# THUDM/GRAND-plus

Measured on AMD Instinct MI355X. Metric: propagation-matrix rows/sec (whole node), higher is better.
Workload: dtype f64

## Files before the change

### grand_plus_amd/csrc/gfpush.hip

```cpp
#include "gfpush_kernels.hpp"
#include "gfpush_sketch.hpp"
#include "gfpush_plan.hpp"
#include "grandplus.h"

#include <dlfcn.h>
#include <sys/prctl.h>
#include <rccl/rccl.h>

#include <algorithm>
#include <atomic>
#include <cmath>
#include <cstdarg>
#include <cstdio>
#include <cstdlib>
#include <cstring>
#include <new>
#include <string>
#include <chrono>
#include <thread>
#include <type_traits>
#include <vector>

using namespace gp;
using namespace gp::planning;
// ... 508 lines not shown
        if (rc == GP_ERR_NOMEM && sk.use && !shape.insists_on_sketch()) {
            sk.use = false; g_last_error.clear();
            continue;
        }
        return rc;
    }
}

KParams call_params(const gp_graph* g, const CallArgs& a, const GeneralPlan& gk, u64* counters)
{
    KParams kp;
    std::memset(&kp, 0, sizeof kp);
    kp.indptr = g->d_indptr; kp.indices = g->d_indices; kp.n_nodes = (int)g->n_nodes; kp.nnz = (int)g->nnz;
    kp.deg_shift = g->deg_shift; kp.node_mask = g->node_mask; kp.deg_sat = g->deg_sat;
    kp.seeds = a.d_seeds; kp.n_seeds = a.n_seeds;
    kp.coef = g->d_coef; kp.n_coef = a.n_coef; kp.rmax = a.rmax; kp.K = a.K;
    kp.out_row = a.d_row; kp.out_col = a.d_col; kp.out_val = a.d_val; kp.out_filled = a.d_filled;
    kp.counters = counters;
    kp.lds_slots = gk.lds_slots;
    kp.force_global = g->opt.force_global;
    kp.prune = prune_allowed(g->opt, a.coef, a.n_coef) ? 1 : 0;
    kp.diag_flags = g->opt.diag_flags;
    kp.rows_distinct = g->rows_distinct && g->opt.seedrow ? 1u : 0u;
    kp.solo = (g->opt.solo_levels ? 1u : 0u) | (g->opt.sk_seed_merge ? 2u : 0u);
    kp.direct = direct_tables(g->opt, g->n_nodes, gk) ? 1 : 0;
    return kp;
}

struct GeneralPass { const u32* rows; int n_rows; int queue; u32* overflow; int n_overflow; int overflow_queue; const u32* order; };

int launch_general(const gp_graph* g, KParams& kp, const GeneralPlan& gk, bool gk_acsr, const GeneralPass& pass, hipStream_t s)
{
    const Workspace& w = g->ws;
    const bool two_tier = w.big.n_wg > 0;
    use_csr(kp, g, gk_acsr, true);
    use_slabs(kp, w.est);
    kp.row_map = pass.rows ? pass.rows : pass.order; kp.n_rows_dev = pass.rows ? kp.counters + pass.n_rows : nullptr; kp.queue_counter = pass.queue;
    kp.retry_list = two_tier ? pass.overflow : nullptr; kp.retry_counter = pass.n_overflow;
    const Kernel k = pass.rows ? retry_kernel(gk.block_threads) : general_kernel(gk.block_threads);
    int rc = launch_kernel(k, gk.block_threads, kp, gk.n_wg, gk.lds_bytes + g->opt.lds_pad, s);
    if (rc || !two_tier) return rc;
    use_slabs(kp, w.big);
    kp.row_map = pass.overflow; kp.n_rows_dev = kp.counters + pass.n_overflow; kp.queue_counter = pass.overflow_queue;
    kp.retry_list = nullptr;
    return launch_kernel(retry_kernel(gk.block_threads), gk.block_threads, kp, w.big.n_wg, gk.lds_bytes + g->opt.lds_pad, s);
}

// ... 383 lines not shown
    if (k == "block_threads") {
        if (value != 256 && value != 512 && value != 768 && value != 1024) return fail(GP_ERR_INVALID_ARG, "block_threads must be 256, 512, 768 or 1024");
        g->opt.block_threads = (int)value;
    } else if (k == "lds_bytes") {
        if (value < 40 * 1024 || value > 160 * 1024) return fail(GP_ERR_INVALID_ARG, "lds_bytes must be in [40960, 163840]");
        g->opt.lds_bytes = (int)(value & ~15ll);
    } else if (k == "lds_pad") {
        if (value < 0 || value > 120 * 1024) return fail(GP_ERR_INVALID_ARG, "lds_pad must be in [0, 122880]");
        g->opt.lds_pad = (int)(value & ~15ll);
    } else if (k == "kernel") {
        if (value < 0 || value > 2) return fail(GP_ERR_INVALID_ARG, "kernel must be 0 (automatic), 1 (general) or 2 (sketch)");
        g->opt.kernel = (int)value;
    } else if (k == "sk_block_threads") {
        if (value != 0 && value != 512 && value != 768 && value != 1024) return fail(GP_ERR_INVALID_ARG, "sk_block_threads must be 0, 512, 768 or 1024");
        g->opt.sk_block = (int)value;
    } else if (k == "sk_lg_mu" || k == "sk_lg_mr") {
        if (value != 0 && (value < 8 || value > 14)) return fail(GP_ERR_INVALID_ARG, "%s must be 0 or in [8, 14]", key);
        (k == "sk_lg_mu" ? g->opt.sk_lg_mu : g->opt.sk_lg_mr) = (int)value;
    } else if (k == "sk_direct_max") {
        if (value < 0 || value > (1 << 20)) return fail(GP_ERR_INVALID_ARG, "sk_direct_max must be in [0, 2^20]");
        g->opt.sk_direct_max = (int)value;
    } else if (k == "sk_seed_merge") {
        g->opt.sk_seed_merge = value ? 1 : 0;
    } else if (k == "row_order") {
        g->opt.row_order = value ? 1 : 0;
    } else if (k == "gk_acsr") {
        g->opt.gk_acsr = value ? 1 : 0;
    } else if (k == "sk_target") {
        if (value < 0 || value > 4096) return fail(GP_ERR_INVALID_ARG, "sk_target must be in [0, 4096]");
        g->opt.sk_target = (int)value;
    } else if (k == "measure_choice") {
        g->opt.measure_choice = value ? 1 : 0;
        if (!value) g->choices.clear();
    } else if (k == "verify_merge") {
        g->opt.verify_merge = value ? 1 : 0;
    } else if (k == "pretouch") {
        g->opt.pretouch = value ? 1 : 0;
    } else if (k == "max_workgroups") {
        if (value < 0 || value > 65535) return fail(GP_ERR_INVALID_ARG, "max_workgroups must be in [0, 65535]");
        g->opt.max_workgroups = (int)value;
    } else if (k == "workspace_mb") {
        if (value < 1) return fail(GP_ERR_INVALID_ARG, "workspace_mb must be >= 1");
        g->opt.workspace_mb = value;
    } else if (k == "est_level_edges") {
        if (value < 0) return fail(GP_ERR_INVALID_ARG, "est_level_edges must be >= 0");
        g->opt.est_level_edges = value;
// ... 230 lines not shown
}

namespace {

int replicate_part(gp_graph* g, int d) {
    gp_graph* src = g->part[0];
    HIP_TRY(hipSetDevice(src->device));
    int rc = ensure_packed(src, src->stream);
    if (rc) return rc;
    HIP_TRY(hipStreamSynchronize(src->stream));
    const int dev = g->devices[d];
    HIP_TRY(hipSetDevice(dev));
    hipDeviceProp_t prop;
    HIP_TRY(hipGetDeviceProperties(&prop, dev));
    gp_graph* q = new (std::nothrow) gp_graph();
    if (!q) return fail(GP_ERR_NOMEM, "host allocation failed");
    struct Guard { gp_graph* q; ~Guard() { if (q) gp_graph_destroy(q); } } guard{q};
    q->device = dev; q->n_nodes = src->n_nodes; q->nnz = src->nnz; q->num_cus = prop.multiProcessorCount;
    q->deg_shift = src->deg_shift; q->node_mask = src->node_mask; q->deg_sat = src->deg_sat;
    q->packed = true; q->opt.max_degree_bits = src->opt.max_degree_bits; q->rows_distinct = src->rows_distinct;
    q->opt.block_threads = src->opt.block_threads; q->opt.lds_bytes = src->opt.lds_bytes; q->opt.max_workgroups = src->opt.max_workgroups;
    q->opt.workspace_mb = src->opt.workspace_mb; q->opt.force_global = src->opt.force_global; q->opt.exact_stats = src->opt.exact_stats;
    q->opt.direct_tables = src->opt.direct_tables; q->opt.est_level_edges = src->opt.est_level_edges; q->opt.seedrow = src->opt.seedrow; q->opt.solo_levels = src->opt.solo_levels;
    q->opt.kernel = src->opt.kernel; q->opt.row_order = src->opt.row_order; q->opt.gk_acsr = src->opt.gk_acsr; q->opt.sk_seed_merge = src->opt.sk_seed_merge; q->opt.sk_block = src->opt.sk_block; q->opt.sk_lg_mu = src->opt.sk_lg_mu; q->opt.sk_lg_mr = src->opt.sk_lg_mr; q->opt.sk_target = src->opt.sk_target; q->opt.lds_pad = src->opt.lds_pad; q->opt.sk_direct_max = src->opt.sk_direct_max;
    const size_t b_ptr = sizeof(int) * (size_t)(q->n_nodes + 1), b_idx = sizeof(int) * (size_t)(q->nnz + 1);
    HIP_TRY(hipMalloc(&q->d_indptr, b_ptr));
    HIP_TRY(hipMalloc(&q->d_indices, b_idx));
    if (dev == src->device) {
        HIP_TRY(hipMemcpy(q->d_indptr, src->d_indptr, b_ptr, hipMemcpyDeviceToDevice));
        HIP_TRY(hipMemcpy(q->d_indices, src->d_indices, b_idx, hipMemcpyDeviceToDevice));
    } else {
        HIP_TRY(hipMemcpyPeer(q->d_indptr, dev, src->d_indptr, src->device, b_ptr));
        HIP_TRY(hipMemcpyPeer(q->d_indices, dev, src->d_indices, src->device, b_idx));
    }
    HIP_TRY(hipMalloc(&q->d_counters, sizeof(u64) * kNumCounters));
    HIP_TRY(hipHostMalloc(&q->h_counters, sizeof(u64) * kNumCounters));
    HIP_TRY(hipEventCreate(&q->ev0));
    HIP_TRY(hipEventCreate(&q->ev1));
    HIP_TRY(hipStreamCreateWithFlags(&q->stream, hipStreamNonBlocking));
    guard.q = nullptr;
    g->part[d] = q;
    return GP_OK;
}

int gfpush_multi(gp_graph* g, const int32_t* seeds, int64_t n_seeds, const double* coef, int n_coef, double rmax, int K,
                 int32_t* row_idx, int32_t* col_idx, double* value)
{
// ... 114 lines not shown
```

### grand_plus_amd/csrc/gfpush_kernels.hpp

```cpp
#pragma once

#include <hip/hip_runtime.h>
#include <stdint.h>

#include "gfpush_hash.hpp"

namespace gp {

typedef unsigned long long u64;
typedef unsigned int u32;

#define GP_LDS  __attribute__((address_space(3)))
#define GP_KARG __attribute__((address_space(4)))
template <class T> __device__ __forceinline__ T* lds_at(u32 byte_off) { return (T*)(GP_LDS T*)(uintptr_t)byte_off; }
__device__ __forceinline__ u32 uni(u32 x) { return (u32)__builtin_amdgcn_readfirstlane((int)x); }
__device__ __forceinline__ int uni(int x) { return __builtin_amdgcn_readfirstlane(x); }
__device__ __forceinline__ u64 uni(u64 x) { return ((u64)uni((u32)(x >> 32)) << 32) | uni((u32)x); }
__device__ __forceinline__ long long uni(long long x) { return (long long)uni((u64)x); }
__device__ __forceinline__ double uni(double x) {
    const u64 b = (u64)__double_as_longlong(x);
    return __longlong_as_double((long long)(((u64)uni((u32)(b >> 32)) << 32) | uni((u32)b)));
}

constexpr int    kEmpty      = -1;
// ... 110 lines not shown
    x += (u32)__builtin_amdgcn_update_dpp(0, (int)x, 0x143, 0xC, 0xF, false);
    return x;
}
__device__ __forceinline__ u32 wave_id() { return (u32)__builtin_amdgcn_readfirstlane((int)(threadIdx.x >> 6)); }
__device__ __forceinline__ u32 wave_sum32(u32 x) {
    return (u32)__builtin_amdgcn_readlane((int)wave_incl_scan_dpp(x), 63);
}

enum Counter { kQueue = 0, kQueueRetry, kRetryRows,
               kQueueRetry2, kRetryRows2,
               kSkSlabFails,
               kMaxLevelEdges, kMaxLogRecords,
               kRetriedTotal,
               kPushes, kEdges, kFilled, kSupport, kFrontier, kLdsLevels,
               kGlobalLevels, kFailedRows, kDegLookups,
               kSkCandEdges, kSkSweep2,
               kTicksScan, kTicksExpand, kTicksTopk, kTicksTotal, kTicksScanHbm, kTicksExpandHbm,
               kDiag0, kDiagLast = kDiag0 + 15,
               kDiagX0, kDiagXLast = kDiagX0 + 255,
               kNumCounters };

enum OvfCount { kOvfLevel = 8,
                kOvfSolo = 9,
                kOvfTopk = 10 };
#if !defined(GP_DIAG) && !defined(GP_SK_TIMING)
#define GP_OVF_COUNT(p, which) __hip_atomic_fetch_add(&(p).counters[kDiag0 + (which)], 1ull, __ATOMIC_RELAXED, __HIP_MEMORY_SCOPE_AGENT)
#else
#define GP_OVF_COUNT(p, which) do { } while (0)
#endif

#ifdef GP_DIAG_HEAVY
constexpr int kSyncBase = __COUNTER__;
#define GP_SYNC() do { constexpr int site_ = (__COUNTER__ - kSyncBase - 1) & 63; const u64 tb_ = clock64(); __syncthreads(); if ((threadIdx.x & 63) == 0) { const u64 w_ = clock64() - tb_; ctl->barw[threadIdx.x >> 6] += w_; ++ctl->barn[threadIdx.x >> 6]; \
    __hip_atomic_fetch_add(&ctl->site_w[site_], w_, __ATOMIC_RELAXED, __HIP_MEMORY_SCOPE_WORKGROUP); __hip_atomic_fetch_add(&ctl->site_n[site_], 1u, __ATOMIC_RELAXED, __HIP_MEMORY_SCOPE_WORKGROUP); } } while (0)
#else
#define GP_SYNC() __syncthreads()
#endif
#ifdef GP_DIAG
#define GP_STAMP(var) do { if (threadIdx.x == 0) var = wall_clock64(); } while (0)
#define GP_ACCUM(acc, t0, t1) do { if (threadIdx.x == 0) acc += (t1) - (t0); } while (0)
#define GP_SUB_BEGIN() do { if (threadIdx.x == 0) gp_sub_t = wall_clock64(); } while (0)
#define GP_SUB(i) do { if (threadIdx.x == 0) { const u64 n_ = wall_clock64(); gp_sub_acc[i] += n_ - gp_sub_t; gp_sub_t = n_; } } while (0)
#define GP_SUB_COUNT(i, n) do { if (threadIdx.x == 0) gp_sub_acc[i] += (n); } while (0)
#else
#define GP_STAMP(var) do { } while (0)
#define GP_ACCUM(acc, t0, t1) do { } while (0)
#define GP_SUB_BEGIN() do { } while (0)
// ... 315 lines not shown
              [se0] "=&v"(se0), [se1] "=&v"(se1), [se2] "=&v"(se2), [se3] "=&v"(se3),
              [sv] "=&s"(sv), [m0] "=&s"(m0), [m1] "=&s"(m1), [m2] "=&s"(m2), [m3] "=&s"(m3), [st] "=&s"(st)
            : [c0] "v"(col[0]), [c1] "v"(col[1]), [c2] "v"(col[2]), [c3] "v"(col[3]), [s0] "v"(sh[0]), [s1] "v"(sh[1]), [s2] "v"(sh[2]), [s3] "v"(sh[3]),
              [emp] "v"(kEmpty), [parts] "s"(parts), [part] "s"(part),
              [capm] "s"(cap - kProbeSpan), [kb] "s"(lds_addr(keys)), [vb] "s"(lds_addr(vals)), [fa] "s"(lds_addr(flag)), [lim] "n"(kMaxProbe)
            : "vcc", "scc", "memory");
    } else {
        u64 ent;
        asm volatile(
            "s_mov_b64 %[sv], exec\n\t"
            GP_IW4_HASHES
            GP_IW4_EACH(GP_IW4_ISSUE_C)
            GP_IW4_RESOLVE_C(0, 3) GP_IW4_RESOLVE_C(1, 2) GP_IW4_RESOLVE_C(2, 1) GP_IW4_RESOLVE_C(3, 0)
            : [sl0] "=&v"(sl0), [sl1] "=&v"(sl1), [sl2] "=&v"(sl2), [sl3] "=&v"(sl3),
              [se0] "=&v"(se0), [se1] "=&v"(se1), [se2] "=&v"(se2), [se3] "=&v"(se3),
              [sv] "=&s"(sv), [ent] "=&s"(ent), [st] "=&s"(st)
            : [c0] "v"(col[0]), [c1] "v"(col[1]), [c2] "v"(col[2]), [c3] "v"(col[3]), [s0] "v"(sh[0]), [s1] "v"(sh[1]), [s2] "v"(sh[2]), [s3] "v"(sh[3]),
              [emp] "v"(kEmpty),
              [capm] "s"(cap - kProbeSpan), [kb] "s"(lds_addr(keys)), [vb] "s"(lds_addr(vals)), [fa] "s"(lds_addr(flag)), [lim] "n"(kMaxProbe)
            : "vcc", "scc", "memory");
    }
}


#define GP_IW2_EACH(X) X(0) X(1)
__device__ __forceinline__ void insert_windows2_asm(int* keys, double* vals, u32 cap, u32* flag, int c0, int c1, double s0, double s1)
{
    u32 sl0, sl1, se0, se1, st; u64 sv, ent;
    asm volatile(
        "s_mov_b64 %[sv], exec\n\t"
        GP_IW2_EACH(GP_IW4_H1) GP_IW2_EACH(GP_IW4_H2) GP_IW2_EACH(GP_IW4_H3) GP_IW2_EACH(GP_IW4_H4)
        GP_IW2_EACH(GP_IW4_ISSUE_C)
        GP_IW4_RESOLVE_C(0, 1) GP_IW4_RESOLVE_C(1, 0)
        : [sl0] "=&v"(sl0), [sl1] "=&v"(sl1), [se0] "=&v"(se0), [se1] "=&v"(se1), [sv] "=&s"(sv), [ent] "=&s"(ent), [st] "=&s"(st)
        : [c0] "v"(c0), [c1] "v"(c1), [s0] "v"(s0), [s1] "v"(s1), [emp] "v"(kEmpty),
          [capm] "s"(cap - kProbeSpan), [kb] "s"(lds_addr(keys)), [vb] "s"(lds_addr(vals)), [fa] "s"(lds_addr(flag)), [lim] "n"(kMaxProbe)
        : "vcc", "scc", "memory");
}

struct SerialSection {
    __device__ __forceinline__ SerialSection() { __builtin_amdgcn_s_setprio(3); }
    __device__ __forceinline__ ~SerialSection() { __builtin_amdgcn_s_setprio(0); }
};

__device__ __forceinline__ void insert_window_solo(int* keys, double* vals, u32 cap, u32* flag, int col, double sh, u32& slot, int& seen)
{
// ... 1772 lines not shown
```

### grand_plus_amd/csrc/gfpush_plan.hpp

```cpp
#pragma once

#include <algorithm>
#include <atomic>
#include <cmath>
#include <cstddef>
#include <cstdint>
#include <cstdio>
#include <cstring>
#include <string>

namespace gp {
namespace planning {

typedef unsigned long long cap_t;

enum Status { kOk = 0, kInvalidArg, kNoMem, kNeedOccupancy };

struct KernelConsts {
    int ctl_bytes = 0, three_lds = 0, min_cap = 0, topk_bins = 0, bucket_cap = 0, unit_shift = 0;
    int sk_max_pushers = 0, sk_max_coef = 0, sk_tie = 0;
};

struct Options {
    int block_threads = 0; int lds_bytes = 0; int max_workgroups = 0;
    int verify_merge = 0;
    int lds_pad = 0; int pretouch = 0;
    int64_t workspace_mb = 65536; int force_global = 0; int exact_stats = 0; int diag_flags = 0; int direct_tables = 1; int seedrow = 1; int solo_levels = 1;
    int kernel = 0;
    int sk_block = 0, sk_lg_mu = 0, sk_lg_mr = 0, sk_target = 0, sk_direct_max = 0;
    int row_order = 1;
    int sk_seed_merge = 1; int gk_acsr = 1;
    int64_t est_level_edges = 0;
    int measure_choice = 1;
    int max_degree_bits = 31;
};

struct Estimate {
    int kind = 0; int last_kind = 1;
    bool sk_auto_off = false; double sk_off_rmax = 0.0; int sk_off_n_coef = 0;
    bool last_sk_soft = false;
    double edges = 0.0, log = 0.0;
    double rmax = -1.0; int n_coef = 0;
    bool recipe_changed = false;
    double cur_edges = 0.0, cur_log = 0.0;
    int64_t last_call_rows = 0; bool grown_for_call = true;
};


struct SlabCaps {
    int n_wg = 0;
    cap_t push_cap = 0, resg_cap = 0, log_cap = 0, cand_cap = 0, bucket_cap = 0, bt_cap = 0;
    cap_t arch_cap = 0;
    size_t log_bytes() const { return arch_cap ? 6 * (size_t)log_cap + 8 * (size_t)arch_cap : 12 * (size_t)log_cap; }
    size_t per_wg() const { return 16 * (size_t)(2 * push_cap + resg_cap + cand_cap + bucket_cap) + log_bytes() + 8 * (size_t)bt_cap + 64; }
// ... 431 lines not shown
```

### grand_plus_amd/csrc/gfpush_sketch.hpp

```cpp
#pragma once

#include "gfpush_kernels.hpp"

#ifndef GP_DIAG

namespace gp {

#ifndef GP_SK_SWEEP_DEPTH
#define GP_SK_SWEEP_DEPTH 2
#endif
constexpr int kSkMaxCoef = 40;
constexpr u32 kSkTie     = 256;

struct CtlS {
    long long row;
    LevelCtr lc[2];
    u32 ovf;
    u32 fail;
    u32 n_sel, n_tie;
    u32 tk_bin, tk_above, tk_count, tk_total;
    u32 tk_t, tk_wide, tk_dig;
    u64 kth_bits;
    u32 bcnt[64];
    u64 st[8], st_row[8];
    double coef[kSkMaxCoef + 1];
    u32 cand_q[kSkMaxCoef];
    int seed_key; u32 tot_pu, tot_log;
    double lv_dang; u32 lv_has_dang;
    u32 max_e, max_log;
    u32 k_log_cap, k_pu_cap, k_direct_max, k_solo_ok, k_cx, k_pad; double k_rscale;
#ifdef GP_SK_TIMING
    u64 tacc[16]; u64 tlast;
    u64 tacc2[14]; u64 tlast2;
    u64 t_enter, t_row, row_sum, row_max;
    u64 row_hist[32];
#endif
};
#ifdef GP_SK_TIMING
#define SKT_BEGIN(ctl) do { if (threadIdx.x == 0) (ctl)->tlast = wall_clock64(); } while (0)
#define SKT(ctl, i) do { if (threadIdx.x == 0) { const u64 n_ = wall_clock64(); (ctl)->tacc[i] += n_ - (ctl)->tlast; (ctl)->tlast = n_; } } while (0)
#define SKT_COUNT(ctl, i, n) do { if (threadIdx.x == 0) (ctl)->tacc[i] += (n); } while (0)
#define SKT2_BEGIN(ctl) do { if (threadIdx.x == 0) (ctl)->tlast2 = wall_clock64(); } while (0)
#define SKT2(ctl, i) do { if (threadIdx.x == 0) { const u64 n_ = wall_clock64(); (ctl)->tacc2[i] += n_ - (ctl)->tlast2; (ctl)->tlast2 = n_; } } while (0)
#else
#define SKT_BEGIN(ctl) do { } while (0)
#define SKT(ctl, i) do { } while (0)
#define SKT_COUNT(ctl, i, n) do { } while (0)
#define SKT2_BEGIN(ctl) do { } while (0)
#define SKT2(ctl, i) do { } while (0)
#endif
static_assert(sizeof(CtlS) <= (size_t)kCtlStruct, "the control block must fit its LDS reservation");
enum StatS { zPush = 0, zEdges, zDeg, zFilled, zLevels, zFailed, zCand, zSweep2, zNumStats };
__device__ __forceinline__ void zstat(CtlS* ctl, int which, u64 n) {
// ... 107 lines not shown
        const u32 i = min(g0 + 4u * lane, last_chunk);
        if (NT) { kn = __builtin_nontemporal_load((const i4*)&lk[i]); pn = __builtin_nontemporal_load((const u2*)&lp[i]); }
        else    { kn = *(const i4*)&lk[i]; pn = *(const u2*)&lp[i]; }
    };
    load(g);
    for (;;) {
        int k[4]; u32 pu[4];
        const u32 i0 = g + 4u * lane;
        const bool whole = g >= first && g + 256u <= end;
        if (whole) {
#pragma unroll
            for (int q = 0; q < 4; ++q) { k[q] = kn[q]; pu[q] = (pn[q >> 1] >> (16 * (q & 1))) & 0xFFFFu; }
        } else {
#pragma unroll
            for (int q = 0; q < 4; ++q) {
                const bool in = i0 + (u32)q >= first && i0 + (u32)q < end;
                k[q] = in ? kn[q] : -1;
                pu[q] = in ? (pn[q >> 1] >> (16 * (q & 1))) & 0xFFFFu : 0u;
            }
        }
        g += kStride;
        const bool more = g < end;
        if (more) load(g);
        if (whole) f(k, pu, SkAllValid<true>()); else f(k, pu, SkAllValid<false>());
        if (!more) break;
    }
}

template <int BLOCK, class F>
__device__ __forceinline__ void log_groups2_nt(const int* lk, const unsigned short* lp, u32 end, F f)
{
    typedef int i4 __attribute__((ext_vector_type(4)));
    typedef u32 u2 __attribute__((ext_vector_type(2)));
    constexpr u32 kStride = (BLOCK / 64) * 256u;
    const u32 lane = threadIdx.x & 63u;
    u32 g = wave_id() * 256u;
    if (g >= end) return;
    const u32 last_chunk = (end - 1u) & ~3u;
    i4 ka, kb; u2 pa, pb;
    auto load = [&](u32 g0, i4& kn, u2& pn) {
        const u32 i = min(g0 + 4u * lane, last_chunk);
        kn = __builtin_nontemporal_load((const i4*)&lk[i]); pn = __builtin_nontemporal_load((const u2*)&lp[i]);
    };
    auto consume = [&](u32 g0, const i4& kn, const u2& pn, int (&k)[4], u32 (&pu)[4]) -> bool {
        const u32 i0 = g0 + 4u * lane;
        const bool whole = g0 + 256u <= end;
        if (whole) {
#pragma unroll
            for (int q = 0; q < 4; ++q) { k[q] = kn[q]; pu[q] = (pn[q >> 1] >> (16 * (q & 1))) & 0xFFFFu; }
        } else {
#pragma unroll
            for (int q = 0; q < 4; ++q) {
                const bool in = i0 + (u32)q < end;
                k[q] = in ? kn[q] : -1;
                pu[q] = in ? (pn[q >> 1] >> (16 * (q & 1))) & 0xFFFFu : 0u;
            }
        }
        return whole;
    };
    load(g, ka, pa);
    kb = ka; pb = pa;
    if (g + kStride < end) load(g + kStride, kb, pb);
    for (;;) {
        int k[4]; u32 pu[4];
        consume(g, ka, pa, k, pu);
        if (g + 2u * kStride < end) load(g + 2u * kStride, ka, pa);
        f(k, pu, SkAllValid<false>());
        g += kStride;
        if (g >= end) break;
        consume(g, kb, pb, k, pu);
        if (g + 2u * kStride < end) load(g + 2u * kStride, kb, pb);
        f(k, pu, SkAllValid<false>());
        g += kStride;
        if (g >= end) break;
    }
}

template <int BLOCK, bool NT, int FX, class F>
__device__ __forceinline__ void sk_edge_stream(KP p, CtlS* ctl, const PushEntry* push, const u32* bt, u32 n_ent, u32 E, double* S,
                                               unsigned short* lp, u32 pu_base, double cs, F f)
{
    constexpr u32 kWaves = BLOCK / 64;
    static_assert(kFlatW == 4, "sk_edge_stream reads the four window flags of a lane as one 32-bit word");
    const u32 lane = threadIdx.x & 63u;
    const u32 wave = wave_id();
    unsigned char* wscr = (unsigned char*)ctl + kCtlStruct + 64 * kFlatW * wave;
    const int* indices = p.indices;
    const u32 sentinel = (u32)p.nnz;
    const u32 units = (E + (1u << kUnitShift) - 1u) >> kUnitShift;
    const u32 slot = kWaves - 1u - wave;
    const u32 u_lo = (slot * units) / kWaves, u_hi = ((slot + 1u) * units) / kWaves;
    if (u_lo >= u_hi || n_ent == 0) return;
    const bool small = n_ent <= 64u;
    u32 btv = 0, bt_first = 0;
    auto load_bt = [&](u32 step0) {
// ... 152 lines not shown
        const double dang = w.ctl->lv_dang; const int seed_key = w.ctl->seed_key;
        if (MODE != 3) {
            lk[E] = seed_key; lp[E] = (unsigned short)(pu_base + n_ent);
            const u32 h = sk_cell((u32)seed_key);
            if (cs != 0.0) lds_add_u32(&w.R[h >> w.shR], fx_up(dang * cs));
            if (MODE == 0) { lds_add_u32(&w.U[h >> w.shU], fx_up(dang * 2147483648.0)); S[n_ent] = dang; }
        }
        if ((MODE == 1 || (MODE == 3 && (parts == 1u || slot_of(hash_b((u32)seed_key), parts) == part))) &&
            !sk_res_add_lds(w.xkeys, w.xvals, capx, seed_key, dang)) w.ctl->ovf = 1;
    }
}

template <int BLOCK>
__device__ GP_PHASE_NOINLINE void phase_sk_filter(u32 lds0, u32 seg_base, u32 n, u32 capx, u32 pu_base, u32 parts, u32 part)
{
    KP p = kparams();
    lds0 = uni(lds0); seg_base = uni(seg_base); n = uni(n); capx = uni(capx); pu_base = uni(pu_base); parts = uni(parts); part = uni(part);
    const SkView w = sk_view<BLOCK>(p, lds0);
    const float thr = p.sk_thr_f;
    const u32 dshift = (u32)p.deg_shift;
    const double* S = w.xvals + capx;
    u32 n_cand = 0;
    SKT2(w.ctl, 0);
    log_groups<BLOCK>(w.log_key, w.log_pu, seg_base, seg_base + n, [&](const int (&k)[4], const u32 (&pu)[4], auto all_valid) {
        constexpr bool kAll = decltype(all_valid)::value;
        u32 cell[4]; double s[4];
#pragma unroll
        for (int q = 0; q < 4; ++q) {
            cell[q] = w.U[sk_cell(kAll ? (u32)k[q] : (u32)max(k[q], 0)) >> w.shU];
            s[q] = S[kAll || k[q] >= 0 ? pu[q] - pu_base : 0u];
        }
        int kc[4];
#pragma unroll
        for (int q = 0; q < 4; ++q) {
            const u32 dq = (u32)k[q] >> dshift;
            const bool cand = (kAll || k[q] >= 0) && (float)cell[q] >= (float)dq * thr;
            n_cand += (u32)__popcll(__ballot(cand));
            kc[q] = cand ? k[q] : -1;
        }
        insert_windows4_asm<true>(w.xkeys, w.xvals, capx, &w.ctl->ovf, kc, s, parts, part);
    });
    if ((threadIdx.x & 63u) == 0 && n_cand && part == 0u) zstat(w.ctl, zCand, n_cand);
    SKT2(w.ctl, 1);
}

template <int BLOCK>
__device__ GP_PHASE_NOINLINE void phase_sk_scan(u32 lds0, u32 cap, u32 nx_sel, u32 nxt_sel, u32 clear_n, u32 pu_next, double cnext)
// ... 344 lines not shown
                if (__ballot(kk[j] != kEmpty && v[j] > 0.0) == 0) continue;
                bool is_sel = false, is_t = false;
                Cand cd; cd.bits = (u64)__double_as_longlong(v[j]); cd.key = kk[j]; cd.pad = 0;
                if (kk[j] != kEmpty && v[j] > 0.0) {
                    const u32 id = (u32)cd.key & p.node_mask;
                    const u64 vbits = cd.bits >> vshift;
                    const bool v_eq = vbits == vpre;
                    const bool in_bin = v_eq && (ishift >= 32u || (id >> ishift) == ipre);
                    const bool over = vbits > vpre || (v_eq && ishift < 32u && (id >> ishift) < ipre);
                    is_sel = over || (in_bin && take_all); is_t = in_bin && !take_all;
                }
                const u32 si = wave_alloc1(&ctl->n_sel, is_sel, lane);
                if (is_sel) t.sel[si] = cd;
                const u32 ti = wave_alloc1(&ctl->n_tie, is_t, lane);
                if (is_t) t.tie[ti] = cd;
            }
        }
    }
    GP_SYNC();
    sk_rank_selected<BLOCK>(p, ctl, t, need, take_all, my_rank);
    return need;
}

template <int BLOCK, bool TG>
__device__ GP_PHASE_NOINLINE void phase_sk_topk(u32 lds0, u32 row_lo, u32 row_hi, int seed, u32 n_pu, u32 n_log)
{
    KP p = kparams();
    lds0 = uni(lds0); row_lo = uni(row_lo); row_hi = uni(row_hi); seed = uni(seed); n_pu = uni(n_pu); n_log = uni(n_log);
    const SkView w = sk_view<BLOCK>(p, lds0);
    CtlS* ctl = w.ctl;
    const SkTop t = sk_top(p, w, TG ? 0u : n_pu);
    const long long row = (long long)(((u64)row_hi << 32) | row_lo);
    const int tid = threadIdx.x, lane = tid & 63;
    const u32 wave = wave_id();
    const u32 K = (u32)p.K;

    if (!TG) for (u32 i = tid; i < n_pu; i += BLOCK) t.T[i] = w.arch[i];
    for (u32 i = tid; i < 512u; i += BLOCK) t.fine[i] = 0;
    for (u32 i = tid; i < t.CA; i += BLOCK) { t.akeys[i] = kEmpty; t.avals[i] = 0.0; }
    if (tid < 64) ctl->bcnt[tid] = 0;
    if (tid == 0) { ctl->ovf = 0; ctl->tk_t = 1u; ctl->n_sel = 0; ctl->n_tie = 0; ctl->tk_wide = 0; ctl->kth_bits = ~0ull; }
    bool table_ready = true;
    GP_SYNC();
    for (u32 i = tid; i < t.MR; i += BLOCK) {
        const u32 cv = t.R[i];
        if (cv) {
            const u32 fb = __float_as_uint((float)cv);
            lds_add_u32(&t.fine[min(511u, (fb >> 19) - (127u << 4))], 1u);
        }
    }
    GP_SYNC();
    u32 t_c;
    {
        u32 cnt8[8], sum = 0;
#pragma unroll
        for (int j = 0; j < 8; ++j) { cnt8[j] = t.fine[8 * lane + j]; sum += cnt8[j]; }
        const u32 suf = wave_suffix_scan(sum, lane);
        const u64 m = __ballot(suf >= p.sk_target);
        u32 edge = 1u;
        if (m != 0) {
            const int cl = 63 - __builtin_clzll(m);
            u32 acc = suf - sum; int js = 0;
#pragma unroll
            for (int j = 7; j >= 0; --j) { acc += cnt8[j]; if (acc >= p.sk_target) { js = j; break; } }
            const u32 bin = 8u * (u32)cl + (u32)__builtin_amdgcn_readlane(js, cl), e = bin >> 4, mt = 16u + (bin & 15u);
            edge = max(e >= 4u ? mt << (e - 4u) : mt >> (4u - e), 1u);
        }
        t_c = edge;
    }
    SKT(ctl, 7);
    u32 need = 0, my_rank = 0;
    bool last = false;
    for (int round = 0; ; ++round) {
        u32 P = 1;
        for (;;) {
            bool ovf = false;
            for (u32 part = 0; part < P; ++part) {
                const u32 n_run = part == 0 ? 0u : need;
                Cand mine; mine.bits = 0; mine.key = kEmpty; mine.pad = 0;
                if ((u32)tid < n_run) mine = t.sel[tid];
                if (!table_ready) {
                    GP_SYNC();
                    for (u32 i = tid; i < t.CA; i += BLOCK) { t.akeys[i] = kEmpty; t.avals[i] = 0.0; }
                    if (tid < 64) ctl->bcnt[tid] = 0;
                    if (tid == 0) { ctl->n_sel = 0; ctl->n_tie = 0; ctl->tk_wide = 0; ctl->kth_bits = ~0ull; }
                    GP_SYNC();
                }
                table_ready = false;
                if (n_run != 0u) {
                    if (mine.key != kEmpty) { t.akeys[t.CA - 1u - (u32)tid] = mine.key; t.avals[t.CA - 1u - (u32)tid] = __longlong_as_double((long long)mine.bits); }
                    GP_SYNC();
                }
                auto tabled = [&](const int (&k)[4], const u32 (&pu)[4], auto all_valid) {
                    constexpr bool kAll = decltype(all_valid)::value;
                    u32 cell[4]; double cv[4];
#pragma unroll
                    for (int q = 0; q < 4; ++q) {
                        cell[q] = t.R[sk_cell(kAll ? (u32)k[q] : (u32)max(k[q], 0)) >> t.shR];
                        cv[q] = TG ? w.arch[pu[q]] : t.T[pu[q]];
                    }
                    int kh[4];
#pragma unroll
                    for (int q = 0; q < 4; ++q) kh[q] = (kAll || k[q] >= 0) && cv[q] != 0.0 && cell[q] >= t_c ? k[q] : -1;
                    insert_windows4_asm<true>(t.akeys, t.avals, t.CA, &ctl->ovf, kh, cv, P, part);
                };
#if GP_SK_SWEEP_DEPTH == 2
                log_groups2_nt<BLOCK>(w.log_key, w.log_pu, n_log, tabled);
#else
                log_groups<BLOCK, true>(w.log_key, w.log_pu, 0u, n_log, tabled);
#endif
                GP_SYNC();
                SKT(ctl, 8);
                if (uni(ctl->ovf)) { ovf = true; break; }
                need = sk_select<BLOCK>(p, ctl, t, my_rank);
                SKT(ctl, 9);
                if (need == 0xFFFFFFFFu) { if (tid == 0) ctl->fail = 3; GP_SYNC(); return; }
            }
            if (!ovf) break;
            GP_SYNC();
            if (tid == 0) { ctl->ovf = 0; GP_OVF_COUNT(p, kOvfTopk); }
            P *= 2; need = 0;
            if (P > 64u) { if (tid == 0) ctl->fail = 4; GP_SYNC(); return; }
            GP_SYNC();
        }
        if (t_c <= 1u || last) break;
        if (need == K) {
            const double tau_fx = __builtin_floor(__longlong_as_double((long long)uni(ctl->kth_bits)) * p.sk_rscale * (1.0 - 1.0 / 1048576.0));
            if (tau_fx >= (double)t_c) break;
            t_c = tau_fx >= 1.0 ? (u32)tau_fx : 1u;
            last = true;
        } else {
            t_c = round >= 2 ? 1u : max(1u, t_c >> 4);
        }
        if (tid == 0) zstat(ctl, zSweep2, 1);
    }
    const long long out0 = row * (long long)p.K;
    if ((u32)tid < need) {
        const Cand cd = t.sel[tid];
        const int node = p.unit_info[(u32)cd.key & p.node_mask];
        __builtin_nontemporal_store(seed, &p.out_row[out0 + my_rank]);
        __builtin_nontemporal_store(node, &p.out_col[out0 + my_rank]);
        __builtin_nontemporal_store(__longlong_as_double((long long)cd.bits), &p.out_val[out0 + my_rank]);
    }
    publish_filled(p, row, need);
// ... 225 lines not shown
    if (tid < 16) ctl->tacc[tid] = 0;
    if (tid < 14) ctl->tacc2[tid] = 0;
    if (tid < 32) ctl->row_hist[tid] = 0;
    if (tid == 0) { ctl->t_enter = wall_clock64(); ctl->row_sum = 0; ctl->row_max = 0; }
#endif
    if (tid < kSkMaxCoef) { ctl->cand_q[tid] = 0; if (tid < p.n_coef) ctl->coef[tid] = p.coef[tid]; }
    if (tid == 0) {
        ctl->max_e = 0; ctl->max_log = 0;
        ctl->k_log_cap = (u32)min(p.log_cap, (u64)0xFFFFFFFFu); ctl->k_pu_cap = (u32)min((u64)kSkMaxPushers, p.arch_cap);
        ctl->k_direct_max = min(p.sk_direct_max, 3u * (w.CX / 4u)); ctl->k_cx = w.CX; ctl->k_rscale = p.sk_rscale;
        ctl->k_solo_ok = (p.solo & 1u) && p.push_cap >= (u64)kSkSoloEdges + 4u &&
                         (double)p.bt_cap >= (p.rmax > 0.0 ? fmin((double)p.nnz, 1.001 / p.rmax + 16.0) : (double)p.nnz) / (double)(1u << kUnitShift) + 4.0 ? 1u : 0u;
    }
    const long long n_rows = p.n_seeds;
    const u32 L = (u32)p.n_coef - 1u;

    for (;;) {
        GP_SYNC();
        SKT_BEGIN(ctl);
        if (tid == 0) {
            long long q = (long long)__hip_atomic_fetch_add(&p.counters[p.queue_counter], 1ull, __ATOMIC_RELAXED, __HIP_MEMORY_SCOPE_AGENT);
            if (p.row_map && q < n_rows) q = (long long)p.row_map[q];
            ctl->row = q;
            ctl->fail = 0; ctl->ovf = 0;
#ifdef GP_SK_TIMING
            ctl->t_row = ctl->tlast;
#endif
        }
        GP_SYNC();
        const long long row = uni(ctl->row);
        if (row >= n_rows) break;
        const int seed = uni(p.seeds[row]);
        if (seed < 0 || seed >= p.n_nodes) {
            if (tid == 0) { __hip_atomic_fetch_add(&ctl->st[zFailed], 1ull, __ATOMIC_RELAXED, __HIP_MEMORY_SCOPE_WORKGROUP); if (p.out_filled) p.out_filled[row] = 0; }
            continue;
        }
        u32 lvl = 1u + uni(phase_sk_seed<BLOCK>(lds0, seed));
        GP_SYNC();
        SKT(ctl, 0); SKT_COUNT(ctl, 15, 1);
        if (lvl == 2u) {
            SKT_COUNT(ctl, 13, 1);
            if (uni(ctl->ovf)) lvl = uni(phase_sk_level1_redo<BLOCK>(lds0, L)) ? 2u : L + 1u;
        }
        for (; lvl <= L; ++lvl)
            if (!uni(phase_sk_level<BLOCK>(lds0, lvl, L))) break;
        GP_SYNC();
        SKT(ctl, 6);
// ... 62 lines not shown
```

Baseline: 3.588 million.

## Spill overflowed top-k inserts to log tail instead of re-sweeping partitions

When the LDS top-k hash table overflows during a sweep, entries that failed to insert are now appended to a spare region after the log in global memory rather than forcing a restart with twice as many hash partitions. After selection, only the spilled entries are re-swept, alternating between two regions. This avoids full re-sweeps of the whole log on overflow. The cost is a wave-level atomic and scattered global writes per failing group, plus a new inline-asm insert variant that returns a per-lane failure mask. It falls back to the old doubling scheme when the spill area is too small.

```diff
diff --git a/grand_plus_amd/csrc/gfpush.hip b/grand_plus_amd/csrc/gfpush.hip
--- a/grand_plus_amd/csrc/gfpush.hip
+++ b/grand_plus_amd/csrc/gfpush.hip
@@ -554,7 +554,7 @@
     kp.prune = prune_allowed(g->opt, a.coef, a.n_coef) ? 1 : 0;
     kp.diag_flags = g->opt.diag_flags;
     kp.rows_distinct = g->rows_distinct && g->opt.seedrow ? 1u : 0u;
-    kp.solo = (g->opt.solo_levels ? 1u : 0u) | (g->opt.sk_seed_merge ? 2u : 0u);
+    kp.solo = (g->opt.solo_levels ? 1u : 0u) | (g->opt.sk_seed_merge ? 2u : 0u) | (g->opt.sk_spill ? 4u : 0u);
     kp.direct = direct_tables(g->opt, g->n_nodes, gk) ? 1 : 0;
     return kp;
 }
@@ -984,6 +984,8 @@
         g->opt.sk_direct_max = (int)value;
     } else if (k == "sk_seed_merge") {
         g->opt.sk_seed_merge = value ? 1 : 0;
+    } else if (k == "sk_spill") {
+        g->opt.sk_spill = value ? 1 : 0;
     } else if (k == "row_order") {
         g->opt.row_order = value ? 1 : 0;
     } else if (k == "gk_acsr") {
@@ -1260,7 +1262,7 @@
     q->opt.block_threads = src->opt.block_threads; q->opt.lds_bytes = src->opt.lds_bytes; q->opt.max_workgroups = src->opt.max_workgroups;
     q->opt.workspace_mb = src->opt.workspace_mb; q->opt.force_global = src->opt.force_global; q->opt.exact_stats = src->opt.exact_stats;
     q->opt.direct_tables = src->opt.direct_tables; q->opt.est_level_edges = src->opt.est_level_edges; q->opt.seedrow = src->opt.seedrow; q->opt.solo_levels = src->opt.solo_levels;
-    q->opt.kernel = src->opt.kernel; q->opt.row_order = src->opt.row_order; q->opt.gk_acsr = src->opt.gk_acsr; q->opt.sk_seed_merge = src->opt.sk_seed_merge; q->opt.sk_block = src->opt.sk_block; q->opt.sk_lg_mu = src->opt.sk_lg_mu; q->opt.sk_lg_mr = src->opt.sk_lg_mr; q->opt.sk_target = src->opt.sk_target; q->opt.lds_pad = src->opt.lds_pad; q->opt.sk_direct_max = src->opt.sk_direct_max;
+    q->opt.kernel = src->opt.kernel; q->opt.row_order = src->opt.row_order; q->opt.gk_acsr = src->opt.gk_acsr; q->opt.sk_seed_merge = src->opt.sk_seed_merge; q->opt.sk_spill = src->opt.sk_spill; q->opt.sk_block = src->opt.sk_block; q->opt.sk_lg_mu = src->opt.sk_lg_mu; q->opt.sk_lg_mr = src->opt.sk_lg_mr; q->opt.sk_target = src->opt.sk_target; q->opt.lds_pad = src->opt.lds_pad; q->opt.sk_direct_max = src->opt.sk_direct_max;
     const size_t b_ptr = sizeof(int) * (size_t)(q->n_nodes + 1), b_idx = sizeof(int) * (size_t)(q->nnz + 1);
     HIP_TRY(hipMalloc(&q->d_indptr, b_ptr));
     HIP_TRY(hipMalloc(&q->d_indices, b_idx));
diff --git a/grand_plus_amd/csrc/gfpush_kernels.hpp b/grand_plus_amd/csrc/gfpush_kernels.hpp
--- a/grand_plus_amd/csrc/gfpush_kernels.hpp
+++ b/grand_plus_amd/csrc/gfpush_kernels.hpp
@@ -156,7 +156,8 @@
 
 enum OvfCount { kOvfLevel = 8,
                 kOvfSolo = 9,
-                kOvfTopk = 10 };
+                kOvfTopk = 10,
+                kOvfSpill = 11 };
 #if !defined(GP_DIAG) && !defined(GP_SK_TIMING)
 #define GP_OVF_COUNT(p, which) __hip_atomic_fetch_add(&(p).counters[kDiag0 + (which)], 1ull, __ATOMIC_RELAXED, __HIP_MEMORY_SCOPE_AGENT)
 #else
@@ -518,6 +519,42 @@
     }
 }
 
+#define GP_IW4_RESOLVE_G(q, cnt) \
+        "s_waitcnt lgkmcnt(" #cnt ")\n\t" \
+        "s_mov_b64 exec, %[m" #q "]\n\t" \
+        GP_IW4_WALK(q) \
+        "s_mov_b64 %[g" #q "], exec\n\t"                           \
+        "s_andn2_b64 exec, %[m" #q "], exec\n\t"                   \
+        "v_lshl_add_u32 %[se" #q "], %[sl" #q "], 3, %[vb]\n\t" \
+        "ds_add_f64 %[se" #q "], %[s" #q "]\n\t"
+__device__ __forceinline__ void insert_windows4_gave_asm(int* keys, double* vals, u32 cap, u32* flag, const int (&col)[4], const double (&sh)[4],
+                                                         u32 parts, u32 part, u64 (&gave)[4])
+{
+    u32 sl0, sl1, sl2, sl3, se0, se1, se2, se3, st; u64 sv;
+    u64 m0, m1, m2, m3, g0, g1, g2, g3;
+    asm volatile(
+        "s_mov_b64 %[sv], exec\n\t"
+        GP_IW4_EACH(GP_IW4_MASK)
+        "s_cmp_eq_u32 %[parts], 1\n\t"
+        "s_cbranch_scc1 4f\n\t"
+        "s_mov_b32 %[st], 0x7feb352d\n\t" GP_IW4_EACH(GP_IW4_F1) GP_IW4_EACH(GP_IW4_F2)
+        "s_mov_b32 %[st], 0x846ca68b\n\t" GP_IW4_EACH(GP_IW4_F3) GP_IW4_EACH(GP_IW4_F4) GP_IW4_EACH(GP_IW4_F5)
+        "4:\n\t"
+        GP_IW4_HASHES
+        GP_IW4_EACH(GP_IW4_ISSUE_M)
+        GP_IW4_RESOLVE_G(0, 3) GP_IW4_RESOLVE_G(1, 2) GP_IW4_RESOLVE_G(2, 1) GP_IW4_RESOLVE_G(3, 0)
+        "s_mov_b64 exec, %[sv]"
+        : [sl0] "=&v"(sl0), [sl1] "=&v"(sl1), [sl2] "=&v"(sl2), [sl3] "=&v"(sl3),
+          [se0] "=&v"(se0), [se1] "=&v"(se1), [se2] "=&v"(se2), [se3] "=&v"(se3),
+          [sv] "=&s"(sv), [m0] "=&s"(m0), [m1] "=&s"(m1), [m2] "=&s"(m2), [m3] "=&s"(m3), [st] "=&s"(st),
+          [g0] "=&s"(g0), [g1] "=&s"(g1), [g2] "=&s"(g2), [g3] "=&s"(g3)
+        : [c0] "v"(col[0]), [c1] "v"(col[1]), [c2] "v"(col[2]), [c3] "v"(col[3]), [s0] "v"(sh[0]), [s1] "v"(sh[1]), [s2] "v"(sh[2]), [s3] "v"(sh[3]),
+          [emp] "v"(kEmpty), [parts] "s"(parts), [part] "s"(part),
+          [capm] "s"(cap - kProbeSpan), [kb] "s"(lds_addr(keys)), [vb] "s"(lds_addr(vals)), [fa] "s"(lds_addr(flag)), [lim] "n"(kMaxProbe)
+        : "vcc", "scc", "memory");
+    gave[0] = g0; gave[1] = g1; gave[2] = g2; gave[3] = g3;
+}
+
 
 #define GP_IW2_EACH(X) X(0) X(1)
 __device__ __forceinline__ void insert_windows2_asm(int* keys, double* vals, u32 cap, u32* flag, int c0, int c1, double s0, double s1)
diff --git a/grand_plus_amd/csrc/gfpush_plan.hpp b/grand_plus_amd/csrc/gfpush_plan.hpp
--- a/grand_plus_amd/csrc/gfpush_plan.hpp
+++ b/grand_plus_amd/csrc/gfpush_plan.hpp
@@ -29,7 +29,7 @@
     int kernel = 0;
     int sk_block = 0, sk_lg_mu = 0, sk_lg_mr = 0, sk_target = 0, sk_direct_max = 0;
     int row_order = 1;
-    int sk_seed_merge = 1; int gk_acsr = 1;
+    int sk_seed_merge = 1; int sk_spill = 1; int gk_acsr = 1;
     int64_t est_level_edges = 0;
     int measure_choice = 1;
     int max_degree_bits = 31;
diff --git a/grand_plus_amd/csrc/gfpush_sketch.hpp b/grand_plus_amd/csrc/gfpush_sketch.hpp
--- a/grand_plus_amd/csrc/gfpush_sketch.hpp
+++ b/grand_plus_amd/csrc/gfpush_sketch.hpp
@@ -1,6 +1,7 @@
 #pragma once
 
 #include "gfpush_kernels.hpp"
+#include "gfpush_spill.hpp"
 
 #ifndef GP_DIAG
 
@@ -29,6 +30,7 @@
     double lv_dang; u32 lv_has_dang;
     u32 max_e, max_log;
     u32 k_log_cap, k_pu_cap, k_direct_max, k_solo_ok, k_cx, k_pad; double k_rscale;
+    u32 sp_n[2];
 #ifdef GP_SK_TIMING
     u64 tacc[16]; u64 tlast;
     u64 tacc2[14]; u64 tlast2;
@@ -182,19 +184,19 @@
         g += kStride;
         const bool more = g < end;
         if (more) load(g);
-        if (whole) f(k, pu, SkAllValid<true>()); else f(k, pu, SkAllValid<false>());
+        if (whole) f(k, pu, SkAllValid<true>(), g - kStride); else f(k, pu, SkAllValid<false>(), g - kStride);
         if (!more) break;
     }
 }
 
 template <int BLOCK, class F>
-__device__ __forceinline__ void log_groups2_nt(const int* lk, const unsigned short* lp, u32 end, F f)
+__device__ __forceinline__ void log_groups2_nt(const int* lk, const unsigned short* lp, u32 first, u32 end, F f)
 {
     typedef int i4 __attribute__((ext_vector_type(4)));
     typedef u32 u2 __attribute__((ext_vector_type(2)));
     constexpr u32 kStride = (BLOCK / 64) * 256u;
     const u32 lane = threadIdx.x & 63u;
-    u32 g = wave_id() * 256u;
+    u32 g = (first & ~3u) + wave_id() * 256u;
     if (g >= end) return;
     const u32 last_chunk = (end - 1u) & ~3u;
     i4 ka, kb; u2 pa, pb;
@@ -204,14 +206,14 @@
     };
     auto consume = [&](u32 g0, const i4& kn, const u2& pn, int (&k)[4], u32 (&pu)[4]) -> bool {
         const u32 i0 = g0 + 4u * lane;
-        const bool whole = g0 + 256u <= end;
+        const bool whole = g0 >= first && g0 + 256u <= end;
         if (whole) {
 #pragma unroll
             for (int q = 0; q < 4; ++q) { k[q] = kn[q]; pu[q] = (pn[q >> 1] >> (16 * (q & 1))) & 0xFFFFu; }
         } else {
 #pragma unroll
             for (int q = 0; q < 4; ++q) {
-                const bool in = i0 + (u32)q < end;
+                const bool in = i0 + (u32)q >= first && i0 + (u32)q < end;
                 k[q] = in ? kn[q] : -1;
                 pu[q] = in ? (pn[q >> 1] >> (16 * (q & 1))) & 0xFFFFu : 0u;
             }
@@ -225,12 +227,12 @@
         int k[4]; u32 pu[4];
         consume(g, ka, pa, k, pu);
         if (g + 2u * kStride < end) load(g + 2u * kStride, ka, pa);
-        f(k, pu, SkAllValid<false>());
+        f(k, pu, SkAllValid<false>(), g);
         g += kStride;
         if (g >= end) break;
         consume(g, kb, pb, k, pu);
         if (g + 2u * kStride < end) load(g + 2u * kStride, kb, pb);
-        f(k, pu, SkAllValid<false>());
+        f(k, pu, SkAllValid<false>(), g);
         g += kStride;
         if (g >= end) break;
     }
@@ -429,7 +431,7 @@
     const double* S = w.xvals + capx;
     u32 n_cand = 0;
     SKT2(w.ctl, 0);
-    log_groups<BLOCK>(w.log_key, w.log_pu, seg_base, seg_base + n, [&](const int (&k)[4], const u32 (&pu)[4], auto all_valid) {
+    log_groups<BLOCK>(w.log_key, w.log_pu, seg_base, seg_base + n, [&](const int (&k)[4], const u32 (&pu)[4], auto all_valid, u32) {
         constexpr bool kAll = decltype(all_valid)::value;
         u32 cell[4]; double s[4];
 #pragma unroll
@@ -820,6 +822,21 @@
     return need;
 }
 
+__device__ __forceinline__ void sk_spill_append(u32* ctr, int* lk, unsigned short* lp, u32 cap, const u64 (&gave)[4], const int (&k)[4], const unsigned short* lp_group)
+{
+    const u32 lane = threadIdx.x & 63u;
+    const u32 tot = (u32)__popcll(gave[0]) + (u32)__popcll(gave[1]) + (u32)__popcll(gave[2]) + (u32)__popcll(gave[3]);
+    u32 base = 0;
+    if (lane == 0) base = __hip_atomic_fetch_add(ctr, tot, __ATOMIC_RELAXED, __HIP_MEMORY_SCOPE_WORKGROUP);
+    base = (u32)__builtin_amdgcn_readfirstlane((int)base);
+#pragma unroll
+    for (int q = 0; q < 4; ++q) {
+        const u32 idx = base + lane_prefix(gave[q]);
+        if (((gave[q] >> lane) & 1ull) != 0 && idx < cap) { lk[idx] = k[q]; lp[idx] = lp_group[4u * lane + (u32)q]; }
+        base += (u32)__popcll(gave[q]);
+    }
+}
+
 template <int BLOCK, bool TG>
 __device__ GP_PHASE_NOINLINE void phase_sk_topk(u32 lds0, u32 row_lo, u32 row_hi, int seed, u32 n_pu, u32 n_log)
 {
@@ -832,6 +849,8 @@
     const int tid = threadIdx.x, lane = tid & 63;
     const u32 wave = wave_id();
     const u32 K = (u32)p.K;
+    const bool spill_on = (p.solo & 4u) != 0u;
+    const u32 klc = uni(ctl->k_log_cap);
 
     if (!TG) for (u32 i = tid; i < n_pu; i += BLOCK) t.T[i] = w.arch[i];
     for (u32 i = tid; i < 512u; i += BLOCK) t.fine[i] = 0;
@@ -871,10 +890,15 @@
     bool last = false;
     for (int round = 0; ; ++round) {
         u32 P = 1;
+        u32 s_first = 0, s_end = n_log;
+        u32 gen = 0, n_first = 0;
         for (;;) {
             bool ovf = false;
             for (u32 part = 0; part < P; ++part) {
-                const u32 n_run = part == 0 ? 0u : need;
+                const bool spilling = spill_on && P == 1u;
+                SkSpillArea ar; ar.start = 0; ar.cap = 0;
+                if (spilling) ar = sk_spill_area(n_log, klc, gen, n_first);
+                const u32 n_run = part == 0 && gen == 0u ? 0u : need;
                 Cand mine; mine.bits = 0; mine.key = kEmpty; mine.pad = 0;
                 if ((u32)tid < n_run) mine = t.sel[tid];
                 if (!table_ready) {
@@ -889,7 +913,7 @@
                     if (mine.key != kEmpty) { t.akeys[t.CA - 1u - (u32)tid] = mine.key; t.avals[t.CA - 1u - (u32)tid] = __longlong_as_double((long long)mine.bits); }
                     GP_SYNC();
                 }
-                auto tabled = [&](const int (&k)[4], const u32 (&pu)[4], auto all_valid) {
+                auto tabled = [&](const int (&k)[4], const u32 (&pu)[4], auto all_valid, u32 g0) {
                     constexpr bool kAll = decltype(all_valid)::value;
                     u32 cell[4]; double cv[4];
 #pragma unroll
@@ -900,24 +924,38 @@
                     int kh[4];
 #pragma unroll
                     for (int q = 0; q < 4; ++q) kh[q] = (kAll || k[q] >= 0) && cv[q] != 0.0 && cell[q] >= t_c ? k[q] : -1;
-                    insert_windows4_asm<true>(t.akeys, t.avals, t.CA, &ctl->ovf, kh, cv, P, part);
+                    u64 gave[4];
+                    insert_windows4_gave_asm(t.akeys, t.avals, t.CA, &ctl->ovf, kh, cv, P, part, gave);
+                    if (spilling && (gave[0] | gave[1] | gave[2] | gave[3]) != 0)
+                        sk_spill_append(&ctl->sp_n[gen & 1u], w.log_key + ar.start, w.log_pu + ar.start, ar.cap, gave, kh, w.log_pu + g0);
                 };
 #if GP_SK_SWEEP_DEPTH == 2
-                log_groups2_nt<BLOCK>(w.log_key, w.log_pu, n_log, tabled);
+                log_groups2_nt<BLOCK>(w.log_key, w.log_pu, s_first, s_end, tabled);
 #else
-                log_groups<BLOCK, true>(w.log_key, w.log_pu, 0u, n_log, tabled);
+                log_groups<BLOCK, true>(w.log_key, w.log_pu, s_first, s_end, tabled);
 #endif
                 GP_SYNC();
                 SKT(ctl, 8);
-                if (uni(ctl->ovf)) { ovf = true; break; }
+                const u32 n_sp = spilling ? uni(ctl->sp_n[gen & 1u]) : 0u;
+                if (spilling) {
+                    if (!sk_spill_fits(ar, n_sp)) { ovf = true; break; }
+                    if (tid == 0 && n_sp != 0u) ctl->ovf = 0;
+                } else if (uni(ctl->ovf)) { ovf = true; break; }
                 need = sk_select<BLOCK>(p, ctl, t, my_rank);
                 SKT(ctl, 9);
                 if (need == 0xFFFFFFFFu) { if (tid == 0) ctl->fail = 3; GP_SYNC(); return; }
+                if (n_sp != 0u) {
+                    if (tid == 0) { ctl->sp_n[gen & 1u] = 0; GP_OVF_COUNT(p, kOvfTopk); GP_OVF_COUNT(p, kOvfSpill); }
+                    if (gen == 0u) n_first = n_sp;
+                    s_first = ar.start; s_end = ar.start + n_sp; ++gen;
+                    part = ~0u;
+                }
             }
             if (!ovf) break;
             GP_SYNC();
-            if (tid == 0) { ctl->ovf = 0; GP_OVF_COUNT(p, kOvfTopk); }
+            if (tid == 0) { ctl->ovf = 0; ctl->sp_n[0] = 0; ctl->sp_n[1] = 0; GP_OVF_COUNT(p, kOvfTopk); }
             P *= 2; need = 0;
+            s_first = 0; s_end = n_log; gen = 0;
             if (P > 64u) { if (tid == 0) ctl->fail = 4; GP_SYNC(); return; }
             GP_SYNC();
         }
@@ -1189,7 +1227,7 @@
             long long q = (long long)__hip_atomic_fetch_add(&p.counters[p.queue_counter], 1ull, __ATOMIC_RELAXED, __HIP_MEMORY_SCOPE_AGENT);
             if (p.row_map && q < n_rows) q = (long long)p.row_map[q];
             ctl->row = q;
-            ctl->fail = 0; ctl->ovf = 0;
+            ctl->fail = 0; ctl->ovf = 0; ctl->sp_n[0] = 0; ctl->sp_n[1] = 0;
 #ifdef GP_SK_TIMING
             ctl->t_row = ctl->tlast;
 #endif
diff --git a/grand_plus_amd/csrc/gfpush_spill.hpp b/grand_plus_amd/csrc/gfpush_spill.hpp
--- /dev/null
+++ b/grand_plus_amd/csrc/gfpush_spill.hpp
@@ -0,0 +1,22 @@
+#pragma once
+
+#include "gfpush_hash.hpp"
+
+namespace gp {
+
+struct SkSpillArea { uint32_t start, cap; };
+
+GP_HD SkSpillArea sk_spill_area(uint32_t used_end, uint32_t log_cap, uint32_t gen, uint32_t n_first) {
+    SkSpillArea a; a.start = 0; a.cap = 0;
+    const uint64_t lo = ((uint64_t)used_end + 3u) & ~(uint64_t)3u, hi = (uint64_t)log_cap & ~(uint64_t)3u;
+    if (lo >= hi) return a;
+    if (gen == 0u) { a.start = (uint32_t)lo; a.cap = (uint32_t)(hi - lo); return a; }
+    const uint64_t mid = lo + (((uint64_t)n_first + 3u) & ~(uint64_t)3u);
+    if (mid > hi) return a;
+    if (gen & 1u) { a.start = (uint32_t)mid; a.cap = (uint32_t)(hi - mid); }
+    else          { a.start = (uint32_t)lo;  a.cap = (uint32_t)(mid - lo); }
+    return a;
+}
+GP_HD bool sk_spill_fits(SkSpillArea a, uint32_t n) { return n <= a.cap; }
+
+}
```

After: 3.578 million. No clear change (-0.3%).
